# supabase/etl

Measured on AMD Instinct MI355X. Metric: WAL bytes/s decoded, higher is better.
Workload: dtype u8; 1 GPU; cfg2_fixed_5xint4: 64 MiB batches of CopyData-framed pgoutput, device-resident in / device-resident out, offsets sidecar, NO_CONTROL | ASYNC; batch_bytes=67108819, frames_per_batch=594511, pool_batches=6, parallelism=shard1

## Files before the change

### etl_amd/csrc/frames.hip.h

```cpp
#pragma once
#include "values.hip.h"

namespace etlg {

DEV void record_error(const DecParams& p, uint32_t frame, uint32_t rank, uint32_t code) {
  unsigned long long key = ((unsigned long long)frame << 16) | ((unsigned long long)rank << 8) | code;
  atomicMin(&p.res->first_err, key);
}

DEV bool load_carry(DecParams& p) {
  if (!p.carry) return true;
  const bool ok = (p.carry->fused_fail & ~2u) == 0 && p.carry->first_err == kNoErr;
  p.in_txn = p.carry->out_in_txn; p.final_lsn = p.carry->out_final_lsn; p.next_ord = p.carry->out_next_ord;
  if (!ok && blockIdx.x == 0 && threadIdx.x == 0) atomicOr(&p.res->fused_fail, 8u);
  return ok;
}

DEV uint32_t slot_host_id(const DecParams& p, int sl) { return sl >= 0 ? p.slots[sl].host_id : (uint32_t)sl; }

DEV void block_scan3_excl(uint32_t& a, uint32_t& b, uint32_t& c, uint32_t* lds, uint32_t tot[3]) {
  const int lane = threadIdx.x & 63, wave = threadIdx.x >> 6, nw = (int)(blockDim.x >> 6);
  const uint32_t ia = wave_scan_add(a), ib = wave_scan_add(b), ic = wave_scan_add(c);
  if (lane == 63) { lds[3 * wave] = ia; lds[3 * wave + 1] = ib; lds[3 * wave + 2] = ic; }
  __syncthreads();
  uint32_t pa = 0, pb = 0, pc = 0, ta = 0, tb = 0, tc = 0;
  for (int w = 0; w < nw; w++) {
    const uint32_t xa = lds[3 * w], xb = lds[3 * w + 1], xc = lds[3 * w + 2];
    if (w < wave) { pa += xa; pb += xb; pc += xc; }
    ta += xa; tb += xb; tc += xc;
  }
  __syncthreads();
  a = pa + ia - a; b = pb + ib - b; c = pc + ic - c;
  tot[0] = ta; tot[1] = tb; tot[2] = tc;
}

// ... 502 lines not shown
```

### etl_amd/csrc/plan.hip

```cpp
#include "lookback.hip.h"

#ifndef ETLG_PLAN_MINWAVES
#define ETLG_PLAN_MINWAVES 5
#endif

namespace etlg {

struct WinLds {
  const ETLG_LDS_AS u8* base;
  DEV uint32_t w(uint32_t aoff) const { return ETLG_LDS_LD32(base + aoff); }
};
struct WinGlb {
  const u8* base; uint32_t lim;
  DEV uint32_t w(uint32_t aoff) const {
    uint32_t v = 0;
    if (aoff + 4 <= lim) __builtin_memcpy(&v, base + aoff, 4);
    else for (uint32_t k = 0; aoff + k < lim; k++) v |= (uint32_t)base[aoff + k] << (8 * k);
    return v;
  }
};
template <class M> DEV uint32_t rd32(const M& m, uint32_t off) {
  const uint32_t a = off & ~3u, s = off & 3u;
  return __builtin_amdgcn_alignbyte(m.w(a + 4), m.w(a), s);
}
// ... 45 lines not shown
    const uint32_t d2 = dig4(pad_word(__builtin_amdgcn_alignbyte(w3, w2, s), k, 2), bad);
    mag = (uint64_t)d0 * 100000000ull + (d1 * 10000u + d2);
    uint64_t lim;
    if (cls == ETLG_TC_U32) lim = 0xFFFFFFFFull;
    else if (cls == ETLG_TC_I16) lim = neg ? 0x8000ull : 0x7FFFull;
    else lim = neg ? 0x80000000ull : 0x7FFFFFFFull;
    ok = (n != 0u) & (nd != 0u) & (n <= 12u) & (nd <= 11u) & (bad == 0u) & (mag <= lim) & ((cls != ETLG_TC_U32) | (neg ^ 1u));
  }
  return neg ? 0 - mag : mag;
}

DEV int plan_find(const PlanParams& q, uint32_t rel_u) {
  const ETLG_CONST_AS uint32_t* t = (const ETLG_CONST_AS uint32_t*)(uintptr_t)q.tabs;
  int lo = 0, hi = (int)q.n_tabs - 1;
  while (lo <= hi) {
    const int mid = (lo + hi) >> 1;
    const uint32_t v = t[mid * (int)(sizeof(PlanTab) / 4)];
    if (v == rel_u) return mid;
    if (v < rel_u) lo = mid + 1; else hi = mid - 1;
  }
  return -1;
}

#define WSTAMP(k) do { if ((q.dbg & 64u) && threadIdx.x == 0) ((unsigned long long*)p.heap)[(size_t)blockIdx.x * 8 + (k)] = wall_clock64(); } while (0)
#define PSTAMP(k) do { if ((q.dbg & 32u) && threadIdx.x == 0 && (blockIdx.x & 15u) == 3u) { const unsigned long long t_ = clock64(); atomicAdd(&p.res->dbg_t[k], t_ - tprev); tprev = t_; } } while (0)

constexpr uint32_t kPreBeginLen = kBodyOff + 20u, kPreCommitLen = kBodyOff + 25u;
constexpr int kPreTilesPerWave = 8, kPreWaves = 8;
constexpr uint32_t pre_log2(uint32_t v) { return v <= 1u ? 0u : 1u + pre_log2(v >> 1); }
constexpr uint32_t kPreGroupLog = pre_log2(kPreTilesPerWave * kPreWaves);
static_assert((1u << kPreGroupLog) == (uint32_t)(kPreTilesPerWave * kPreWaves), "a group of the pre-pass is a power of two of tiles");
static_assert(kPreTilesPerWave <= 32 && kPreWaves <= 8, "cand_m / short_m are 32-bit masks; at most two waves per SIMD");
constexpr uint32_t kPlanMaxPolls = 1u << 15;

struct PlanPre2 { unsigned long long a0 = 0, l0 = 0, a1 = 0, l1 = 0; bool valid = false; };
struct PlanFold { uint32_t fx, mk, l0, l1; };
DEV PlanFold fold_id() { return PlanFold{0u, 0u, 0u, 0u}; }
DEV PlanFold fold_f(const PlanFold& a, const PlanFold& b) {
  return PlanFold{a.fx + b.fx, a.mk > b.mk ? a.mk : b.mk, b.mk ? b.l0 : a.l0, b.mk ? b.l1 : a.l1};
}
DEV PlanFold fold_of(unsigned long long a, unsigned long long l) {
  return PlanFold{(uint32_t)a, (uint32_t)(a >> 32) & 0x3FFFFFFFu, (uint32_t)l, (uint32_t)(l >> 32) & 0x3FFFFFFFu};
}
DEV unsigned long long fold_agg(const PlanFold& v) { return ((unsigned long long)v.mk << 32) | v.fx; }
DEV unsigned long long fold_lsn(const PlanFold& v) { return ((unsigned long long)v.l1 << 32) | v.l0; }
DEV unsigned long long pair_state(unsigned long long a, unsigned long long l) { const unsigned long long st = a & ST_MASK; return st == (l & ST_MASK) ? st : 0ull; }
DEV PlanFold fold_scan(PlanFold v) {
#define ETLG_P3_DPP(ctrl, rmask) { PlanFold o_; \
// ... 69 lines not shown
    const PlanFold wfold = fold_lane63(fold_scan((int)lane >= (first_incl < 0 ? 0 : first_incl) ? fold_of(wa, wl) : fold_id()));
    acc = fold_f(wfold, acc);
    if (first_incl >= 0) break;
    base -= 64;
  }
  if (j == 63u && lane == 0) { const PlanFold incl = fold_f(acc, group_agg); ETLG_ST_PAIR(g2 + 2 * (size_t)g, ST_INCL | fold_agg(incl), ST_INCL | fold_lsn(incl)); }
  const PlanFold r = fold_f(acc, local);
  ex = fold_agg(r); ex_lsn = fold_lsn(r);
}

template <int RD>
struct PlanLocal {
  uint32_t tbl, slot_id, pm, x_fx, fixed_dw, vbytes, bad;
  uint32_t tagf;
  uint64_t wal_start, b_lsn;
  uint32_t* rimg;
  uint32_t row[RD];
  uint64_t ord;
  uint64_t agg, tile_lsn, ex, ex_lsn, tile_pre_lsn;
  uint32_t tot_mark, tot_fx;
  bool early, done;
};

template <class M, int RD>
DEV void plan_local(const DecParams& p, const PlanParams& q, const M& m, u8* rows, bool stage_own, uint32_t a0, uint32_t tile, uint32_t nt, uint32_t my_o,
                    uint32_t span0, uint32_t span1, unsigned long long& tprev, PlanLocal<RD>& L, bool keep) {
  L.done = true;
  const uint32_t lane = threadIdx.x;
  const bool live = lane < nt;
  const uint32_t f = tile * 64u + lane;
  uint32_t* failp = &p.res->fused_fail;
  uint32_t bad = 0;

  const uint32_t o0 = my_o;
  const uint32_t o1 = (uint32_t)__builtin_amdgcn_update_dpp((int)span1, (int)my_o, 0x130, 0xF, 0xF, false);
  const uint32_t flen = o1 - o0;
  const uint32_t sane = (live ? 1u : 0u) & (o1 > o0) & (o0 >= span0) & (o1 <= span1) & (flen >= 38u);
  bad |= (live ? 1u : 0u) & (sane ^ 1u);
  const uint32_t fr = sane ? o0 - a0 : 0u;
  const uint64_t h30 = rd64(m, fr + 30);
  const uint32_t tag = (uint32_t)(h30 & 0xFF);
  const uint32_t rel = __builtin_bswap32((uint32_t)(h30 >> 8));
  const uint32_t ncols = ((uint32_t)(h30 >> 48) & 0xFFu) << 8 | (uint32_t)(h30 >> 56);
  bad |= sane & (uint32_t)(tag != 'I' && tag != 'U' && tag != 'D' && tag != 'B' && tag != 'C');
  const bool isD = sane && tag == 'D';
  const bool isI = sane && (tag == 'I' || tag == 'U'), isB = sane && tag == 'B', isC = sane && tag == 'C';
  int ti = -1;
  uint32_t row_dw = 0, slot_id = 0, want_cols = 0, key_dw = 0, n_ident = 0;
// ... 13 lines not shown
    }
  }
  bad |= (uint32_t)(isI && (ti < 0 || ncols != want_cols));
  bad |= (uint32_t)(isD && (ti < 0 || key_dw == 0 || (ncols != n_ident && ncols != want_cols)));
  uint64_t b_lsn = 0;
  if (isB) b_lsn = bswap64(rd64(m, fr + 31));
  if (isC) b_lsn = bswap64(rd64(m, fr + 32));
  const uint32_t fixed_dw = isI ? row_dw : isD ? key_dw : isB ? 2u : isC ? 4u : 0u;
  const uint32_t mark = isB ? (((f + 1) << 1) | 1u) : isC ? ((f + 1) << 1) : 0u;
  const uint32_t im = wave_scan_max(mark);
  const uint32_t pm = (uint32_t)__builtin_amdgcn_update_dpp(0, (int)im, 0x138, 0xF, 0xF, false);
  const uint32_t ifx = wave_scan_add(fixed_dw);
  const uint32_t tot_mark = wave_last(im), tot_fx = wave_last(ifx);
  const uint32_t x_fx = ifx - fixed_dw;
  uint64_t tile_lsn = 0;
  if (tot_mark & 1u) {
    const int src = (int)((tot_mark >> 1) - 1u - tile * 64u);
    tile_lsn = ((uint64_t)(uint32_t)__builtin_amdgcn_readlane((int)(uint32_t)(b_lsn >> 32), src) << 32) | (uint32_t)__builtin_amdgcn_readlane((int)(uint32_t)b_lsn, src);
    bad |= (uint32_t)((tile_lsn >> 62) != 0);
    tile_lsn &= ~(3ull << 62);
  }
  PSTAMP(2);
  WSTAMP(2);
  if (q.dbg & 4u) { if (tot_mark + tot_fx == 0xFFFFFFF1u) atomicOr(failp, 2u); return; }

  const uint64_t agg = ((uint64_t)tot_mark << 32) | tot_fx;
  const bool early = (tile & 63u) == 63u;
  uint64_t ex = 0, ex_lsn = 0;
  if (q.pre) bad |= (uint32_t)((isB && flen != kPreBeginLen) || (isC && flen != kPreCommitLen) || (isI && ti >= 0 && (row_dw != q.pre_row_dw || flen < q.pre_key_below)) ||
                               (isD && ti >= 0 && (key_dw != q.pre_key_dw || (flen >= q.pre_key_below && flen > q.pre_key_max))));
  else plan_publish2(q.desc, tile, agg, tile_lsn);
  if (early && !q.pre) plan_resolve2(q.desc, q.desc + 2 * (size_t)q.ntiles, tile, agg, tile_lsn, failp, PlanPre2(), ex, ex_lsn);
  {
    const uint64_t h0 = rd64(m, fr);
    const uint32_t len = __builtin_bswap32((uint32_t)(h0 >> 8));
    const uint32_t env = ((uint32_t)(h0 & 0xFF) == 'd') & (len + 1u == flen) & ((uint32_t)((h0 >> 40) & 0xFF) == 'w');
    const uint32_t shape = (tag == 'I' || tag == 'U') ? (uint32_t)((uint32_t)((h30 >> 40) & 0xFF) == 'N')
                         : tag == 'D' ? (uint32_t)((uint32_t)((h30 >> 40) & 0xFF) == 'K')
                         : tag == 'B' ? (uint32_t)(flen >= kBodyOff + 20) : (uint32_t)(flen >= kBodyOff + 25);
    bad |= sane & ((env & shape) ^ 1u);
  }
  const uint64_t wal_start = bswap64(rd64(m, fr + 6));
  uint64_t b_ts = 0, c_end = 0;
  uint32_t b_xid = 0, c_flags = 0;
  if (isB) { b_ts = bswap64(rd64(m, fr + 39)); b_xid = __builtin_bswap32(rd32(m, fr + 47)); }
  if (isC) { c_flags = (uint32_t)(h30 >> 8) & 0xFFu; c_end = bswap64(rd64(m, fr + 40)); b_ts = bswap64(rd64(m, fr + 48)); }
  uint32_t* rimg = q.lds_bytes > q.rows_off ? (uint32_t*)(rows + q.rows_off) + x_fx : (uint32_t*)(rows + (stage_own ? ((fr + 3u) & ~3u) : lane * 32u));
  if (isB && !bad) { rimg[0] = (uint32_t)b_ts; rimg[1] = (uint32_t)(b_ts >> 32); }
  if (isC && !bad) { rimg[0] = (uint32_t)c_end; rimg[1] = (uint32_t)(c_end >> 32); rimg[2] = (uint32_t)b_ts; rimg[3] = (uint32_t)(b_ts >> 32); }
  uint32_t vbytes = 0;
  if (!(q.dbg & 8u)) {
    unsigned long long todo = __ballot(isI && !bad);
    while (todo) {
      const int leader = __builtin_ctzll(todo);
      const int t_u = __builtin_amdgcn_readlane(ti, leader);
      const bool mine = isI && !bad && ti == t_u;
      const ETLG_CONST_AS uint32_t* tw = (const ETLG_CONST_AS uint32_t*)(uintptr_t)(q.tabs + t_u);
      const uint32_t n_u = tw[2], cb_u = tw[4];
      const ETLG_CONST_AS uint32_t* cw = (const ETLG_CONST_AS uint32_t*)(uintptr_t)(q.cols + cb_u);
      if (mine) {
        uint32_t cur = fr + 38;
        const uint32_t e = fr + flen;
        uint32_t acc = 0, cbad = 0;
        uint32_t cd_next = cw[0];
        for (uint32_t i = 0; i < n_u; i++) {
          const uint32_t cd = cd_next;
          cd_next = cw[i + 1 < n_u ? i + 1 : i];
          const uint32_t cls = cd & 0xFFu;
          uint32_t* slot = rimg + (cd >> 18);
          const uint32_t rc = cur < e ? cur : fr;
          const uint64_t ch = rd64(m, rc);
          const uint32_t kind = (uint32_t)(ch & 0xFF);
          const uint32_t len = __builtin_bswap32((uint32_t)(ch >> 8));
          const uint32_t c0 = (uint32_t)(ch >> 40) & 0xFFu;
// ... 67 lines not shown
            cbad |= fits ^ 1u;
          }
          vbytes += tl;
          cur = rc + (is_t ? 5u + tl : 1u);
        }
        bad |= cbad;
      }
      todo_d &= ~__ballot(mine);
    }
  }
  PSTAMP(3);
  WSTAMP(3);
  L.tbl = isB ? b_xid : (isI || isD) ? rel : 0u; L.slot_id = (isI || isD) ? slot_id : 0u; L.pm = pm; L.x_fx = x_fx; L.fixed_dw = fixed_dw; L.vbytes = vbytes; L.bad = bad;
  if (isD) c_flags = ETLG_OLD_KEY;
  L.tagf = tag | (c_flags << 8) | (((isI || isD) ? 1u : 0u) << 16) | ((isB ? 1u : 0u) << 17) | ((isC ? 1u : 0u) << 18) | ((live ? 1u : 0u) << 19);
  L.wal_start = wal_start; L.b_lsn = b_lsn; L.rimg = rimg;
  if (keep) {
#pragma unroll
    for (int d = 0; d < RD; d++) L.row[d] = rimg[d];
  }
  L.agg = agg; L.tile_lsn = tile_lsn; L.ex = ex; L.ex_lsn = ex_lsn; L.tot_mark = tot_mark; L.tot_fx = tot_fx; L.early = early; L.done = false;
}

DEV void plan_late_carry(DecParams& p, uint32_t* failp) {
  if (!(p.flags & 16u) || !p.carry) return;
  for (uint32_t polls = 0;; polls++) {
    if (__hip_atomic_load(&p.carry->carry_ready, __ATOMIC_ACQUIRE, __HIP_MEMORY_SCOPE_AGENT)) break;
    if (polls > kPlanMaxPolls) { if (threadIdx.x == 0) atomicOr(failp, 1u); break; }
    __builtin_amdgcn_s_sleep(8);
  }
  p.in_txn = __hip_atomic_load(&p.carry->out_in_txn, __ATOMIC_RELAXED, __HIP_MEMORY_SCOPE_AGENT);
  p.final_lsn = __hip_atomic_load(&p.carry->out_final_lsn, __ATOMIC_RELAXED, __HIP_MEMORY_SCOPE_AGENT);
  p.next_ord = __hip_atomic_load(&p.carry->out_next_ord, __ATOMIC_RELAXED, __HIP_MEMORY_SCOPE_AGENT);
  p.flags &= ~16u;
}

struct PlanPreWords { unsigned long long g0 = 0, g1 = 0, t0 = 0, t1 = 0; };
DEV PlanPreWords plan_pre_load(const PlanParams& q, uint32_t tile) {
  PlanPreWords w;
  if (q.pre && tile < q.ntiles) {
    const ETLG_CONST_AS unsigned long long* dt = (const ETLG_CONST_AS unsigned long long*)(uintptr_t)(q.pre + 2 * (size_t)tile);
    const ETLG_CONST_AS unsigned long long* dg = (const ETLG_CONST_AS unsigned long long*)(uintptr_t)(q.pre + 2 * ((size_t)q.ntiles + (tile >> kPreGroupLog)));
    w.t0 = dt[0]; w.t1 = dt[1]; w.g0 = dg[0]; w.g1 = dg[1];
  }
  return w;
}

template <int RD>
DEV void plan_resolve(DecParams& p, const PlanParams& q, uint32_t tile, PlanLocal<RD>& L, unsigned long long& tprev, const PlanPre2& pre = PlanPre2(), const PlanPreWords& pw = PlanPreWords()) {
  if (L.done) return;
  const uint32_t lane = threadIdx.x;
  const uint32_t f = tile * 64u + lane;
  uint32_t* failp = &p.res->fused_fail;
  uint32_t bad = L.bad;
  const bool isI = (L.tagf >> 16) & 1u, isB = (L.tagf >> 17) & 1u, isC = (L.tagf >> 18) & 1u;
  const uint32_t pm = L.pm;
  const uint64_t b_lsn = L.b_lsn;
  uint64_t ex = L.ex, ex_lsn = L.ex_lsn;

  if (q.pre) {
    const PlanFold r = fold_f(fold_of(pw.g0, pw.g1), fold_of(pw.t0, pw.t1));
    ex = fold_agg(r); ex_lsn = fold_lsn(r);
  }
  else if (!L.early) plan_resolve2(q.desc, q.desc + 2 * (size_t)q.ntiles, tile, L.agg, L.tile_lsn, failp, pre, ex, ex_lsn);
  PSTAMP(7);
  uint32_t pre_mark = (uint32_t)(ex >> 32);
  if (pre_mark == 0) {
    plan_late_carry(p, failp);
    if (p.in_txn) { pre_mark = 1u; ex |= 1ull << 32; }
  }
  const uint64_t pre_lsn = (pre_mark & 1u) && (pre_mark >> 1) != 0 ? ex_lsn : p.final_lsn;
  PSTAMP(4);
  WSTAMP(4);

  const uint32_t last = pre_mark > pm ? pre_mark : pm;
  const bool in_txn = (last & 1u) != 0;
  const uint32_t fb1 = last >> 1;
  uint64_t final_lsn = 0;
  {
    const bool here = in_txn && fb1 != 0 && fb1 - 1 >= tile * 64u;
    const uint32_t src = here ? fb1 - 1 - tile * 64u : 0u;
    const uint32_t lo = (uint32_t)__shfl((int)(uint32_t)b_lsn, (int)src, 64), hi = (uint32_t)__shfl((int)(uint32_t)(b_lsn >> 32), (int)src, 64);
    if (in_txn) final_lsn = here ? (((uint64_t)hi << 32) | lo) : pre_lsn;
  }
  uint64_t ord = 0;
  if (!isB && in_txn) ord = fb1 == 0 ? p.next_ord + f : (uint64_t)(f - (fb1 - 1));
  bad |= (uint32_t)((isI || isC) && !in_txn);
  bad |= (uint32_t)(isC && in_txn && b_lsn != final_lsn);
  L.bad = bad; L.ex = ex; L.tile_pre_lsn = pre_lsn;
  L.b_lsn = isI ? final_lsn : b_lsn;
  L.ord = ord;
}

template <bool REGS, int RD>
DEV void plan_store(DecParams& p, const PlanParams& q, uint32_t tile, const PlanLocal<RD>& L, unsigned long long& tprev) {
  if (L.done) return;
  const uint32_t lane = threadIdx.x;
  const uint32_t f = tile * 64u + lane;
  uint32_t* failp = &p.res->fused_fail;
  const uint32_t bad = L.bad;
  const uint32_t tag = L.tagf & 0xFFu, c_flags = (L.tagf >> 8) & 0xFFu;
  const bool live = (L.tagf >> 19) & 1u;
  const uint32_t x_fx = L.x_fx, fixed_dw = L.fixed_dw, vbytes = L.vbytes, tot_mark = L.tot_mark, tot_fx = L.tot_fx;
  const uint64_t tile_lsn = L.tile_lsn, pre_lsn = L.tile_pre_lsn;
  const uint32_t pre_mark = (uint32_t)(L.ex >> 32);
  const uint64_t pre_fx = (uint64_t)(uint32_t)L.ex << 2;

  if (tile == q.ntiles - 1 && lane == 0) {
    DevResult* r = p.res;
    r->n_events = p.nframes; r->fixed_bytes = pre_fx + ((uint64_t)tot_fx << 2); r->heap_bytes = 0; r->n_frames = p.nframes;
    const uint32_t lm = pre_mark > tot_mark ? pre_mark : tot_mark;
    const bool it = (lm & 1u) != 0;
    r->out_in_txn = it;
    uint64_t fl = 0, no = 0;
    if (it) {
      const uint32_t lb1 = lm >> 1;
      fl = tot_mark ? tile_lsn : pre_lsn;
      no = lb1 == 0 ? p.next_ord + p.nframes : (uint64_t)(p.nframes - (lb1 - 1));
    }
    r->out_final_lsn = fl; r->out_next_ord = no;
    __hip_atomic_store(&r->carry_ready, 1u, __ATOMIC_RELEASE, __HIP_MEMORY_SCOPE_AGENT);
  }

  const uint64_t fx_off = pre_fx + ((uint64_t)x_fx << 2);
  const uint32_t any_bad = __any(bad != 0u) ? 1u : 0u;
  const bool cap_ok = pre_fx + ((uint64_t)tot_fx << 2) <= p.fixed_cap;
  if (!any_bad && cap_ok && !(q.dbg & 8u)) {
    uint32_t* dst = (uint32_t*)(p.fixed + fx_off);
    if (REGS) {
#pragma unroll
      for (uint32_t d = 0; d < (uint32_t)RD; d++) if (d < fixed_dw) dst[d] = L.row[d];
    } else {
      const uint32_t* rimg = L.rimg;
      for (uint32_t d = 0; d < fixed_dw; d++) dst[d] = rimg[d];
    }
  }
  PSTAMP(5);
  if (live && !any_bad && cap_ok && !(q.dbg & 16u)) {
    p.ev_kind[f] = (u8)tag;
    p.ev_flags[f] = (u8)c_flags;
    p.ev_table[f] = L.tbl;
    p.ev_slot[f] = L.slot_id;
    p.ev_start[f] = L.wal_start;
    p.ev_commit[f] = L.b_lsn;
    p.ev_ord[f] = L.ord;
    p.ev_body[f] = fx_off;
  }
  PSTAMP(6);
  WSTAMP(5);
  const bool is_upd = (L.tagf & 0xFFu) == 'U', is_del = (L.tagf & 0xFFu) == 'D';
  const uint32_t pay = wave_last(wave_scan_add((is_upd || is_del) ? 0u : vbytes));
  if (lane == 0 && pay) atomicAdd(&p.res->pay_shard[tile & 31][0], (unsigned long long)pay);
  if (__ballot(is_upd && vbytes != 0)) {
    const uint32_t payu = wave_last(wave_scan_add(is_upd ? vbytes : 0u));
    if (lane == 0 && payu) atomicAdd(&p.res->pay_shard[tile & 31][1], (unsigned long long)payu);
  }
  if (__ballot(is_del && vbytes != 0)) {
    const uint32_t payd = wave_last(wave_scan_add(is_del ? vbytes : 0u));
    if (lane == 0 && payd) atomicAdd(&p.res->pay_shard[tile & 31][2], (unsigned long long)payd);
  }
  if ((any_bad || !cap_ok) && lane == 0) atomicOr(failp, 2u);
}

struct TileSpan { uint32_t nt, span0, span1, my_o; };
DEV TileSpan plan_span(const DecParams& p, uint32_t tile) {
  const uint32_t lane = threadIdx.x;
  TileSpan t;
  const uint32_t f0 = tile * 64u;
  t.nt = p.nframes - f0 < 64u ? p.nframes - f0 : 64u;
  const ETLG_CONST_AS uint32_t* offs_c = (const ETLG_CONST_AS uint32_t*)(uintptr_t)p.offs;
  t.span0 = offs_c[f0]; t.span1 = offs_c[f0 + t.nt];
  t.my_o = lane < t.nt ? p.offs[f0 + lane] : t.span1;
  return t;
}

template <int RD>
DEV void plan_stage_local(DecParams& p, const PlanParams& q, u8* smem, uint32_t tile, const TileSpan& ts, unsigned long long& tprev, PlanLocal<RD>& L, bool keep) {
  const uint32_t lane = threadIdx.x;
  L.done = true;
  const uint32_t nt = ts.nt, span0 = ts.span0, span1 = ts.span1, my_o = ts.my_o;
  PSTAMP(0);
  const uint32_t a0 = span0 & ~15u;
  const bool staged = span1 > span0 && span1 <= p.in_len && (uint64_t)(span1 - a0) + 64 <= q.rows_off && !(q.dbg & 1u);
  if (staged) {
    const uint32_t npieces = (span1 - a0 + 1023u) >> 10;
    for (uint32_t k = 0; k < npieces; k++) {
      const uint32_t c = a0 + (k << 10) + (lane << 4);
      if (c < span1 && (uint64_t)c + 16 <= p.in_len) ETLG_GLDS16(p.in + c, smem + (k << 10));
    }
    const uint32_t tail = a0 + (((uint32_t)p.in_len - a0) & ~15u);
    if (tail < span1 && (uint64_t)tail + 16 > p.in_len && tail + lane < p.in_len && lane < 16) smem[tail - a0 + lane] = p.in[tail + lane];
    ETLG_VMEM_WAIT();
    PSTAMP(1);
    WSTAMP(1);
    if (q.dbg & 2u) { if (smem[lane * 97u] == 0xEE && smem[lane * 13u + 5u] == 0xEF && my_o == 0xFFFFFFF1u) atomicOr(&p.res->fused_fail, 2u); return; }
    const WinLds m{(const ETLG_LDS_AS u8*)smem};
    plan_local(p, q, m, smem, true, a0, tile, nt, my_o, span0, span1, tprev, L, keep);
  } else {
    const WinGlb m{p.in, (uint32_t)p.in_len};
    plan_local(p, q, m, smem, false, 0u, tile, nt, my_o, span0, span1, tprev, L, keep);
  }
}

DEV bool plan_frames_from_device(DecParams& p, PlanParams& q) {
  if (!p.nframes_dev) return true;
  const ETLG_CONST_AS uint32_t* r = (const ETLG_CONST_AS uint32_t*)(uintptr_t)p.nframes_dev;
  const uint32_t nf = r[0], flags = r[1] | r[2];
  if (flags != 0 || nf == 0 || nf > p.nframes) {
    if (blockIdx.x == 0 && threadIdx.x == 0) {
      atomicOr(&p.res->fused_fail, 32u);
      __hip_atomic_store(&p.res->carry_ready, 1u, __ATOMIC_RELEASE, __HIP_MEMORY_SCOPE_AGENT);
    }
    return false;
  }
  p.nframes = nf;
  q.ntiles = (nf + 63u) >> 6;
  return true;
}

template <bool TWO, int RD>
DEV void plan_kernel(DecParams& p, const PlanParams& q_in, u8* smem) {
  PlanParams q = q_in;
  const uint32_t lane = threadIdx.x;
  unsigned long long tprev = (q.dbg & 32u) ? clock64() : 0ull;
  const uint32_t tile = blockIdx.x;
  WSTAMP(0);
  clear_next_descriptors<64>(q.d_clear, q.clear_words, lane);
  if (!(p.flags & 16u) && !load_carry(p)) return;
  if (!plan_frames_from_device(p, q)) return;
  const uint32_t t0 = TWO ? 2u * blockIdx.x : blockIdx.x;
  if (t0 >= q.ntiles) return;
  const TileSpan sa = plan_span(p, t0);
  const PlanPreWords pwa = plan_pre_load(q, t0), pwb = TWO ? plan_pre_load(q, t0 + 1u) : PlanPreWords();
  TileSpan sb = sa;
  if (TWO && t0 + 1u < q.ntiles) sb = plan_span(p, t0 + 1u);
  PlanLocal<RD> A;
  plan_stage_local(p, q, smem, t0, sa, tprev, A, TWO);
  if (TWO) {
    const uint32_t t1 = t0 + 1u;
    PlanLocal<RD> B;
    B.done = true;
    if (t1 < q.ntiles) {
      __threadfence_block();
      __syncthreads();
      plan_stage_local(p, q, smem, t1, sb, tprev, B, false);
    }
    PlanPre2 preA, preB;
    if (!A.done && !A.early && !q.pre) preA = plan_prefetch2(q.desc, q.desc + 2 * (size_t)q.ntiles, t0);
    if (!B.done && !B.early && !q.pre) preB = plan_prefetch2(q.desc, q.desc + 2 * (size_t)q.ntiles, t1);
    plan_resolve(p, q, t0, A, tprev, preA, pwa);
    plan_resolve(p, q, t1, B, tprev, preB, pwb);
    plan_store<true>(p, q, t0, A, tprev);
    plan_store<false>(p, q, t1, B, tprev);
  } else {
    plan_resolve(p, q, t0, A, tprev, PlanPre2(), pwa);
    plan_store<false>(p, q, t0, A, tprev);
  }
}

__global__ __launch_bounds__(kPreWaves * 64) void k_plan_pre(DecParams p, PlanParams q) {
  __shared__ unsigned long long s_wagg[kPreWaves][2];
  if (!plan_frames_from_device(p, q)) return;
  if (blockIdx.x >= ((q.ntiles + (1u << kPreGroupLog) - 1u) >> kPreGroupLog)) return;
  const uint32_t lane = threadIdx.x & 63u, wave = (uint32_t)__builtin_amdgcn_readfirstlane((int)(threadIdx.x >> 6)), g = blockIdx.x;
  const uint32_t t0 = (g << kPreGroupLog) + wave * (uint32_t)kPreTilesPerWave;
  uint32_t o[kPreTilesPerWave + 1];
#pragma unroll
  for (int i = 0; i <= kPreTilesPerWave; i++) {
    const uint64_t f = (uint64_t)(t0 + (uint32_t)i) * 64u + lane;
    o[i] = p.offs[f < p.nframes ? f : p.nframes];
  }
  uint32_t cand_m = 0;
  uint32_t short_m = 0;
  uint32_t tagv[kPreTilesPerWave];
  uint64_t lsnv[kPreTilesPerWave];
#pragma unroll
  for (int i = 0; i < kPreTilesPerWave; i++) {
    const uint64_t f = (uint64_t)(t0 + (uint32_t)i) * 64u + lane;
    const uint32_t o0 = o[i];
// ... 66 lines not shown
    unsigned long long a = gi < ng ? na : tagbits, l = gi < ng ? nl : tagbits;
    if (gi + 64u < ng) ETLG_LD_PAIR(gd + 2 * (size_t)(gi + 64u), na, nl);
    bool have = pair_state(a, l) == tagbits;
    bool gave_up = false;
    for (uint32_t polls = 0;; polls++) {
      if (!have) { ETLG_LD_PAIR(gd + 2 * (size_t)gi, a, l); have = pair_state(a, l) == tagbits; }
      if (!__ballot(!have)) break;
      if (polls > kPlanMaxPolls) { if (lane == 0) atomicOr(&p.res->fused_fail, 1u); gave_up = true; break; }
      __builtin_amdgcn_s_sleep(2);
    }
    const PlanFold inc = fold_scan(gi < ng ? fold_of(a, l) : fold_id());
    PlanFold exc;
    exc.fx = (uint32_t)__builtin_amdgcn_update_dpp(0, (int)inc.fx, 0x138, 0xF, 0xF, false); exc.mk = (uint32_t)__builtin_amdgcn_update_dpp(0, (int)inc.mk, 0x138, 0xF, 0xF, false);
    exc.l0 = (uint32_t)__builtin_amdgcn_update_dpp(0, (int)inc.l0, 0x138, 0xF, 0xF, false); exc.l1 = (uint32_t)__builtin_amdgcn_update_dpp(0, (int)inc.l1, 0x138, 0xF, 0xF, false);
    const PlanFold r = fold_f(carry, exc);
    if (gi < ng && !gave_up) { gd[2 * (size_t)gi] = fold_agg(r); gd[2 * (size_t)gi + 1] = fold_lsn(r); }
    carry = fold_f(carry, fold_lane63(inc));
  }
  if (lane == 0) __hip_atomic_store(q.pre_ticket, 0u, __ATOMIC_RELAXED, __HIP_MEMORY_SCOPE_AGENT);
}

__global__ __launch_bounds__(64, ETLG_PLAN_MINWAVES) void k_plan(DecParams p, PlanParams q) {
  ETLG_DYNAMIC_LDS(smem);
  plan_kernel<false, 1>(p, q, smem);
}

template <int RD>
__global__ __launch_bounds__(64, ETLG_PLAN_MINWAVES) void k_plan2(DecParams p, PlanParams q) {
  ETLG_DYNAMIC_LDS(smem);
  plan_kernel<true, RD>(p, q, smem);
}

}

extern "C" {

using namespace etlg;

void etlg_k_launch_plan_pre(const DecParams* p, const PlanParams* q, hipStream_t s) {
  hipLaunchKernelGGL(k_plan_pre, dim3((q->ntiles + (1u << kPreGroupLog) - 1u) >> kPreGroupLog), dim3(kPreWaves * 64), 0, s, *p, *q);
}

void etlg_k_launch_plan(const DecParams* p, const PlanParams* q, hipStream_t s) {
  if (q->lds_bytes == q->rows_off && q->max_row_dw <= 8u && !(q->dbg & 512u)) {
    if (q->max_row_dw <= 6u) hipLaunchKernelGGL(k_plan2<6>, dim3((q->ntiles + 1) / 2), dim3(64), q->lds_bytes, s, *p, *q);
    else hipLaunchKernelGGL(k_plan2<8>, dim3((q->ntiles + 1) / 2), dim3(64), q->lds_bytes, s, *p, *q);
  } else hipLaunchKernelGGL(k_plan, dim3(q->ntiles), dim3(64), q->lds_bytes, s, *p, *q);
}

uint32_t etlg_k_plan_pre_group_log(void) { return kPreGroupLog; }

int etlg_k_plan_set_lds(void) {
  const int a = hipFuncSetAttribute((const void*)k_plan, hipFuncAttributeMaxDynamicSharedMemorySize, 64 * 1024) == hipSuccess ? 0 : 1;
  const int b = hipFuncSetAttribute((const void*)k_plan2<6>, hipFuncAttributeMaxDynamicSharedMemorySize, 64 * 1024) == hipSuccess ? 0 : 1;
  const int c = hipFuncSetAttribute((const void*)k_plan2<8>, hipFuncAttributeMaxDynamicSharedMemorySize, 64 * 1024) == hipSuccess ? 0 : 1;
  return a | b | c;
}

}
```

Before: 1861 GB/s.

## Split plan kernel into debug and non-debug variants and hoist prologue loads

```diff
diff --git a/etl_amd/csrc/frames.hip.h b/etl_amd/csrc/frames.hip.h
--- a/etl_amd/csrc/frames.hip.h
+++ b/etl_amd/csrc/frames.hip.h
@@ -8,9 +8,10 @@
   atomicMin(&p.res->first_err, key);
 }
 
+DEV bool carry_usable(uint32_t fused_fail, unsigned long long first_err) { return (fused_fail & ~2u) == 0 && first_err == kNoErr; }
 DEV bool load_carry(DecParams& p) {
   if (!p.carry) return true;
-  const bool ok = (p.carry->fused_fail & ~2u) == 0 && p.carry->first_err == kNoErr;
+  const bool ok = carry_usable(p.carry->fused_fail, p.carry->first_err);
   p.in_txn = p.carry->out_in_txn; p.final_lsn = p.carry->out_final_lsn; p.next_ord = p.carry->out_next_ord;
   if (!ok && blockIdx.x == 0 && threadIdx.x == 0) atomicOr(&p.res->fused_fail, 8u);
   return ok;
diff --git a/etl_amd/csrc/plan.hip b/etl_amd/csrc/plan.hip
--- a/etl_amd/csrc/plan.hip
+++ b/etl_amd/csrc/plan.hip
@@ -91,8 +91,11 @@
   return -1;
 }
 
-#define WSTAMP(k) do { if ((q.dbg & 64u) && threadIdx.x == 0) ((unsigned long long*)p.heap)[(size_t)blockIdx.x * 8 + (k)] = wall_clock64(); } while (0)
-#define PSTAMP(k) do { if ((q.dbg & 32u) && threadIdx.x == 0 && (blockIdx.x & 15u) == 3u) { const unsigned long long t_ = clock64(); atomicAdd(&p.res->dbg_t[k], t_ - tprev); tprev = t_; } } while (0)
+template <bool DBG> DEV bool plan_dbg(const PlanParams& q, uint32_t bits) {
+  if constexpr (DBG) return (q.dbg & bits) != 0u; else return false;
+}
+#define WSTAMP(k) do { if constexpr (DBG) { if ((q.dbg & 64u) && threadIdx.x == 0) ((unsigned long long*)p.heap)[(size_t)blockIdx.x * 8 + (k)] = wall_clock64(); } } while (0)
+#define PSTAMP(k) do { if constexpr (DBG) { if ((q.dbg & 32u) && threadIdx.x == 0 && (blockIdx.x & 15u) == 3u) { const unsigned long long t_ = clock64(); atomicAdd(&p.res->dbg_t[k], t_ - tprev); tprev = t_; } } } while (0)
 
 constexpr uint32_t kPreBeginLen = kBodyOff + 20u, kPreCommitLen = kBodyOff + 25u;
 constexpr int kPreTilesPerWave = 8, kPreWaves = 8;
@@ -208,8 +211,8 @@
   bool early, done;
 };
 
-template <class M, int RD>
-DEV void plan_local(const DecParams& p, const PlanParams& q, const M& m, u8* rows, bool stage_own, uint32_t a0, uint32_t tile, uint32_t nt, uint32_t my_o,
+template <bool DBG, class M, int RD>
+DEV void plan_local(const DecParams& p, const PlanParams& q, uint32_t ntiles, const M& m, u8* rows, bool stage_own, uint32_t a0, uint32_t tile, uint32_t nt, uint32_t my_o,
                     uint32_t span0, uint32_t span1, unsigned long long& tprev, PlanLocal<RD>& L, bool keep) {
   L.done = true;
   const uint32_t lane = threadIdx.x;
@@ -269,7 +272,7 @@
   }
   PSTAMP(2);
   WSTAMP(2);
-  if (q.dbg & 4u) { if (tot_mark + tot_fx == 0xFFFFFFF1u) atomicOr(failp, 2u); return; }
+  if (plan_dbg<DBG>(q, 4u)) { if (lane == 0) atomicOr(failp, tot_mark + tot_fx == 0xFFFFFFF1u ? 3u : 2u); return; }
 
   const uint64_t agg = ((uint64_t)tot_mark << 32) | tot_fx;
   const bool early = (tile & 63u) == 63u;
@@ -277,7 +280,7 @@
   if (q.pre) bad |= (uint32_t)((isB && flen != kPreBeginLen) || (isC && flen != kPreCommitLen) || (isI && ti >= 0 && (row_dw != q.pre_row_dw || flen < q.pre_key_below)) ||
                                (isD && ti >= 0 && (key_dw != q.pre_key_dw || (flen >= q.pre_key_below && flen > q.pre_key_max))));
   else plan_publish2(q.desc, tile, agg, tile_lsn);
-  if (early && !q.pre) plan_resolve2(q.desc, q.desc + 2 * (size_t)q.ntiles, tile, agg, tile_lsn, failp, PlanPre2(), ex, ex_lsn);
+  if (early && !q.pre) plan_resolve2(q.desc, q.desc + 2 * (size_t)ntiles, tile, agg, tile_lsn, failp, PlanPre2(), ex, ex_lsn);
   {
     const uint64_t h0 = rd64(m, fr);
     const uint32_t len = __builtin_bswap32((uint32_t)(h0 >> 8));
@@ -296,7 +299,7 @@
   if (isB && !bad) { rimg[0] = (uint32_t)b_ts; rimg[1] = (uint32_t)(b_ts >> 32); }
   if (isC && !bad) { rimg[0] = (uint32_t)c_end; rimg[1] = (uint32_t)(c_end >> 32); rimg[2] = (uint32_t)b_ts; rimg[3] = (uint32_t)(b_ts >> 32); }
   uint32_t vbytes = 0;
-  if (!(q.dbg & 8u)) {
+  if (!plan_dbg<DBG>(q, 8u)) {
     unsigned long long todo = __ballot(isI && !bad);
     while (todo) {
       const int leader = __builtin_ctzll(todo);
@@ -410,32 +413,47 @@
   L.agg = agg; L.tile_lsn = tile_lsn; L.ex = ex; L.ex_lsn = ex_lsn; L.tot_mark = tot_mark; L.tot_fx = tot_fx; L.early = early; L.done = false;
 }
 
-DEV void plan_late_carry(DecParams& p, uint32_t* failp) {
-  if (!(p.flags & 16u) || !p.carry) return;
+struct PlanBatch {
+  uint32_t nframes, ntiles, in_txn;
+  uint64_t final_lsn, next_ord;
+  const DevResult* carry;
+  bool late;
+};
+DEV void plan_late_carry(PlanBatch& b, uint32_t* failp) {
+  if (!b.late) return;
   for (uint32_t polls = 0;; polls++) {
-    if (__hip_atomic_load(&p.carry->carry_ready, __ATOMIC_ACQUIRE, __HIP_MEMORY_SCOPE_AGENT)) break;
+    if (__hip_atomic_load(&b.carry->carry_ready, __ATOMIC_ACQUIRE, __HIP_MEMORY_SCOPE_AGENT)) break;
     if (polls > kPlanMaxPolls) { if (threadIdx.x == 0) atomicOr(failp, 1u); break; }
     __builtin_amdgcn_s_sleep(8);
   }
-  p.in_txn = __hip_atomic_load(&p.carry->out_in_txn, __ATOMIC_RELAXED, __HIP_MEMORY_SCOPE_AGENT);
-  p.final_lsn = __hip_atomic_load(&p.carry->out_final_lsn, __ATOMIC_RELAXED, __HIP_MEMORY_SCOPE_AGENT);
-  p.next_ord = __hip_atomic_load(&p.carry->out_next_ord, __ATOMIC_RELAXED, __HIP_MEMORY_SCOPE_AGENT);
-  p.flags &= ~16u;
+  b.in_txn = __hip_atomic_load(&b.carry->out_in_txn, __ATOMIC_RELAXED, __HIP_MEMORY_SCOPE_AGENT);
+  b.final_lsn = __hip_atomic_load(&b.carry->out_final_lsn, __ATOMIC_RELAXED, __HIP_MEMORY_SCOPE_AGENT);
+  b.next_ord = __hip_atomic_load(&b.carry->out_next_ord, __ATOMIC_RELAXED, __HIP_MEMORY_SCOPE_AGENT);
+  b.late = false;
 }
 
 struct PlanPreWords { unsigned long long g0 = 0, g1 = 0, t0 = 0, t1 = 0; };
-DEV PlanPreWords plan_pre_load(const PlanParams& q, uint32_t tile) {
+DEV uint32_t plan_pre_load(const unsigned long long* pre, uint32_t ntiles, uint32_t tile0) {
+  const uint32_t lane = threadIdx.x, tile = tile0 + (lane >> 3);
+  uint32_t v = 0;
+  if (pre && lane < 16u && tile < ntiles) {
+    const unsigned long long* w = pre + 2 * ((lane & 4u) ? (size_t)ntiles + (tile >> kPreGroupLog) : (size_t)tile);
+    v = ((const uint32_t*)w)[lane & 3u];
+  }
+  return v;
+}
+DEV PlanPreWords plan_pre_words(uint32_t v, int which) {
+  uint32_t d[8];
+#pragma unroll
+  for (int i = 0; i < 8; i++) d[i] = (uint32_t)__builtin_amdgcn_readlane((int)v, 8 * which + i);
   PlanPreWords w;
-  if (q.pre && tile < q.ntiles) {
-    const ETLG_CONST_AS unsigned long long* dt = (const ETLG_CONST_AS unsigned long long*)(uintptr_t)(q.pre + 2 * (size_t)tile);
-    const ETLG_CONST_AS unsigned long long* dg = (const ETLG_CONST_AS unsigned long long*)(uintptr_t)(q.pre + 2 * ((size_t)q.ntiles + (tile >> kPreGroupLog)));
-    w.t0 = dt[0]; w.t1 = dt[1]; w.g0 = dg[0]; w.g1 = dg[1];
-  }
+  w.t0 = ((unsigned long long)d[1] << 32) | d[0]; w.t1 = ((unsigned long long)d[3] << 32) | d[2];
+  w.g0 = ((unsigned long long)d[5] << 32) | d[4]; w.g1 = ((unsigned long long)d[7] << 32) | d[6];
   return w;
 }
 
-template <int RD>
-DEV void plan_resolve(DecParams& p, const PlanParams& q, uint32_t tile, PlanLocal<RD>& L, unsigned long long& tprev, const PlanPre2& pre = PlanPre2(), const PlanPreWords& pw = PlanPreWords()) {
+template <bool DBG, int RD>
+DEV void plan_resolve(const DecParams& p, const PlanParams& q, PlanBatch& b, uint32_t tile, PlanLocal<RD>& L, unsigned long long& tprev, const PlanPre2& pre, uint32_t pre_v, int which) {
   if (L.done) return;
   const uint32_t lane = threadIdx.x;
   const uint32_t f = tile * 64u + lane;
@@ -447,17 +465,18 @@
   uint64_t ex = L.ex, ex_lsn = L.ex_lsn;
 
   if (q.pre) {
+    const PlanPreWords pw = plan_pre_words(pre_v, which);
     const PlanFold r = fold_f(fold_of(pw.g0, pw.g1), fold_of(pw.t0, pw.t1));
     ex = fold_agg(r); ex_lsn = fold_lsn(r);
   }
-  else if (!L.early) plan_resolve2(q.desc, q.desc + 2 * (size_t)q.ntiles, tile, L.agg, L.tile_lsn, failp, pre, ex, ex_lsn);
+  else if (!L.early) plan_resolve2(q.desc, q.desc + 2 * (size_t)b.ntiles, tile, L.agg, L.tile_lsn, failp, pre, ex, ex_lsn);
   PSTAMP(7);
   uint32_t pre_mark = (uint32_t)(ex >> 32);
   if (pre_mark == 0) {
-    plan_late_carry(p, failp);
-    if (p.in_txn) { pre_mark = 1u; ex |= 1ull << 32; }
-  }
-  const uint64_t pre_lsn = (pre_mark & 1u) && (pre_mark >> 1) != 0 ? ex_lsn : p.final_lsn;
+    plan_late_carry(b, failp);
+    if (b.in_txn) { pre_mark = 1u; ex |= 1ull << 32; }
+  }
+  const uint64_t pre_lsn = (pre_mark & 1u) && (pre_mark >> 1) != 0 ? ex_lsn : b.final_lsn;
   PSTAMP(4);
   WSTAMP(4);
 
@@ -472,7 +491,7 @@
     if (in_txn) final_lsn = here ? (((uint64_t)hi << 32) | lo) : pre_lsn;
   }
   uint64_t ord = 0;
-  if (!isB && in_txn) ord = fb1 == 0 ? p.next_ord + f : (uint64_t)(f - (fb1 - 1));
+  if (!isB && in_txn) ord = fb1 == 0 ? b.next_ord + f : (uint64_t)(f - (fb1 - 1));
   bad |= (uint32_t)((isI || isC) && !in_txn);
   bad |= (uint32_t)(isC && in_txn && b_lsn != final_lsn);
   L.bad = bad; L.ex = ex; L.tile_pre_lsn = pre_lsn;
@@ -480,8 +499,8 @@
   L.ord = ord;
 }
 
-template <bool REGS, int RD>
-DEV void plan_store(DecParams& p, const PlanParams& q, uint32_t tile, const PlanLocal<RD>& L, unsigned long long& tprev) {
+template <bool DBG, bool REGS, int RD>
+DEV void plan_store(const DecParams& p, const PlanParams& q, const PlanBatch& b, uint32_t tile, const PlanLocal<RD>& L, unsigned long long& tprev) {
   if (L.done) return;
   const uint32_t lane = threadIdx.x;
   const uint32_t f = tile * 64u + lane;
@@ -494,9 +513,9 @@
   const uint32_t pre_mark = (uint32_t)(L.ex >> 32);
   const uint64_t pre_fx = (uint64_t)(uint32_t)L.ex << 2;
 
-  if (tile == q.ntiles - 1 && lane == 0) {
+  if (tile == b.ntiles - 1 && lane == 0) {
     DevResult* r = p.res;
-    r->n_events = p.nframes; r->fixed_bytes = pre_fx + ((uint64_t)tot_fx << 2); r->heap_bytes = 0; r->n_frames = p.nframes;
+    r->n_events = b.nframes; r->fixed_bytes = pre_fx + ((uint64_t)tot_fx << 2); r->heap_bytes = 0; r->n_frames = b.nframes;
     const uint32_t lm = pre_mark > tot_mark ? pre_mark : tot_mark;
     const bool it = (lm & 1u) != 0;
     r->out_in_txn = it;
@@ -504,7 +523,7 @@
     if (it) {
       const uint32_t lb1 = lm >> 1;
       fl = tot_mark ? tile_lsn : pre_lsn;
-      no = lb1 == 0 ? p.next_ord + p.nframes : (uint64_t)(p.nframes - (lb1 - 1));
+      no = lb1 == 0 ? b.next_ord + b.nframes : (uint64_t)(b.nframes - (lb1 - 1));
     }
     r->out_final_lsn = fl; r->out_next_ord = no;
     __hip_atomic_store(&r->carry_ready, 1u, __ATOMIC_RELEASE, __HIP_MEMORY_SCOPE_AGENT);
@@ -513,7 +532,7 @@
   const uint64_t fx_off = pre_fx + ((uint64_t)x_fx << 2);
   const uint32_t any_bad = __any(bad != 0u) ? 1u : 0u;
   const bool cap_ok = pre_fx + ((uint64_t)tot_fx << 2) <= p.fixed_cap;
-  if (!any_bad && cap_ok && !(q.dbg & 8u)) {
+  if (!any_bad && cap_ok && !plan_dbg<DBG>(q, 8u)) {
     uint32_t* dst = (uint32_t*)(p.fixed + fx_off);
     if (REGS) {
 #pragma unroll
@@ -524,7 +543,7 @@
     }
   }
   PSTAMP(5);
-  if (live && !any_bad && cap_ok && !(q.dbg & 16u)) {
+  if (live && !any_bad && cap_ok && !plan_dbg<DBG>(q, 16u)) {
     p.ev_kind[f] = (u8)tag;
     p.ev_flags[f] = (u8)c_flags;
     p.ev_table[f] = L.tbl;
@@ -550,99 +569,190 @@
   if ((any_bad || !cap_ok) && lane == 0) atomicOr(failp, 2u);
 }
 
+
 struct TileSpan { uint32_t nt, span0, span1, my_o; };
-DEV TileSpan plan_span(const DecParams& p, uint32_t tile) {
+DEV TileSpan plan_span(const uint32_t* offs, uint32_t nframes, uint32_t tile) {
   const uint32_t lane = threadIdx.x;
   TileSpan t;
   const uint32_t f0 = tile * 64u;
-  t.nt = p.nframes - f0 < 64u ? p.nframes - f0 : 64u;
-  const ETLG_CONST_AS uint32_t* offs_c = (const ETLG_CONST_AS uint32_t*)(uintptr_t)p.offs;
+  t.nt = nframes - f0 < 64u ? nframes - f0 : 64u;
+  const ETLG_CONST_AS uint32_t* offs_c = (const ETLG_CONST_AS uint32_t*)(uintptr_t)offs;
   t.span0 = offs_c[f0]; t.span1 = offs_c[f0 + t.nt];
-  t.my_o = lane < t.nt ? p.offs[f0 + lane] : t.span1;
+  t.my_o = offs[f0 + (lane < t.nt ? lane : t.nt)];
   return t;
 }
-
-template <int RD>
-DEV void plan_stage_local(DecParams& p, const PlanParams& q, u8* smem, uint32_t tile, const TileSpan& ts, unsigned long long& tprev, PlanLocal<RD>& L, bool keep) {
+struct TileSpanB { uint32_t nt, ends, my_o; };
+DEV TileSpanB plan_span_b(const uint32_t* offs, uint32_t nframes, uint32_t tile) {
+  const uint32_t lane = threadIdx.x;
+  TileSpanB t;
+  const uint32_t f0 = tile * 64u;
+  t.nt = nframes - f0 < 64u ? nframes - f0 : 64u;
+  t.ends = offs[f0 + (lane ? t.nt : 0u)];
+  t.my_o = offs[f0 + (lane < t.nt ? lane : t.nt)];
+  return t;
+}
+DEV TileSpan plan_span_of(const TileSpanB& s) {
+  return TileSpan{s.nt, (uint32_t)__builtin_amdgcn_readlane((int)s.ends, 0), (uint32_t)__builtin_amdgcn_readlane((int)s.ends, 1), s.my_o};
+}
+
+struct PlanCarry { unsigned long long first_err = kNoErr; uint32_t fused_fail = 0, in_txn = 0; uint64_t final_lsn = 0, next_ord = 0; };
+DEV PlanCarry plan_carry_load(const DevResult* carry) {
+  const ETLG_CONST_AS DevResult* c = (const ETLG_CONST_AS DevResult*)(uintptr_t)carry;
+  PlanCarry w;
+  w.first_err = c->first_err; w.fused_fail = c->fused_fail; w.in_txn = c->out_in_txn; w.final_lsn = c->out_final_lsn; w.next_ord = c->out_next_ord;
+  return w;
+}
+DEV void plan_carry_failed(DevResult* res) { if (blockIdx.x == 0 && threadIdx.x == 0) atomicOr(&res->fused_fail, 8u); }
+
+struct PlanDevCount { uint32_t nf = 0, flags = 0; };
+DEV PlanDevCount plan_count_load(const uint32_t* nframes_dev) {
+  const ETLG_CONST_AS uint32_t* r = (const ETLG_CONST_AS uint32_t*)(uintptr_t)nframes_dev;
+  PlanDevCount c;
+  c.nf = r[0]; c.flags = r[1] | r[2];
+  return c;
+}
+DEV bool plan_count_ok(const PlanDevCount& c, uint32_t bound) { return c.flags == 0 && c.nf != 0 && c.nf <= bound; }
+DEV void plan_count_failed(DevResult* res) {
+  if (blockIdx.x == 0 && threadIdx.x == 0) {
+    atomicOr(&res->fused_fail, 32u);
+    __hip_atomic_store(&res->carry_ready, 1u, __ATOMIC_RELEASE, __HIP_MEMORY_SCOPE_AGENT);
+  }
+}
+DEV bool plan_frames_from_device(DecParams& p, PlanParams& q) {
+  if (!p.nframes_dev) return true;
+  const PlanDevCount c = plan_count_load(p.nframes_dev);
+  if (!plan_count_ok(c, p.nframes)) { plan_count_failed(p.res); return false; }
+  p.nframes = c.nf;
+  q.ntiles = (c.nf + 63u) >> 6;
+  return true;
+}
+
+struct PlanStage { uint32_t a0; bool staged; };
+template <bool DBG>
+DEV PlanStage plan_stage_issue(const DecParams& p, const PlanParams& q, const u8* in, uint64_t in_len, u8* smem, const TileSpan& ts, unsigned long long& tprev) {
+  const uint32_t lane = threadIdx.x;
+  const uint32_t span0 = ts.span0, span1 = ts.span1;
+  PSTAMP(0);
+  PlanStage g;
+  g.a0 = span0 & ~15u;
+  g.staged = span1 > span0 && span1 <= in_len && (uint64_t)(span1 - g.a0) + 64 <= q.rows_off && !plan_dbg<DBG>(q, 1u);
+  if (g.staged) {
+    const uint32_t a0 = g.a0, npieces = (span1 - a0 + 1023u) >> 10;
+    for (uint32_t k = 0; k < npieces; k++) {
+      const uint32_t c = a0 + (k << 10) + (lane << 4);
+      if (c < span1 && (uint64_t)c + 16 <= in_len) ETLG_GLDS16(in + c, smem + (k << 10));
+    }
+    const uint32_t tail = a0 + (((uint32_t)in_len - a0) & ~15u);
+    if (tail < span1 && (uint64_t)tail + 16 > in_len && tail + lane < in_len && lane < 16) smem[tail - a0 + lane] = in[tail + lane];
+  }
+  return g;
+}
+
+template <bool DBG, int RD>
+DEV void plan_stage_local(const DecParams& p, const PlanParams& q, uint32_t ntiles, const u8* in, uint64_t in_len, u8* smem, uint32_t tile, const TileSpan& ts,
+                          const PlanStage& g, unsigned long long& tprev, PlanLocal<RD>& L, bool keep) {
   const uint32_t lane = threadIdx.x;
   L.done = true;
   const uint32_t nt = ts.nt, span0 = ts.span0, span1 = ts.span1, my_o = ts.my_o;
-  PSTAMP(0);
-  const uint32_t a0 = span0 & ~15u;
-  const bool staged = span1 > span0 && span1 <= p.in_len && (uint64_t)(span1 - a0) + 64 <= q.rows_off && !(q.dbg & 1u);
-  if (staged) {
-    const uint32_t npieces = (span1 - a0 + 1023u) >> 10;
-    for (uint32_t k = 0; k < npieces; k++) {
-      const uint32_t c = a0 + (k << 10) + (lane << 4);
-      if (c < span1 && (uint64_t)c + 16 <= p.in_len) ETLG_GLDS16(p.in + c, smem + (k << 10));
-    }
-    const uint32_t tail = a0 + (((uint32_t)p.in_len - a0) & ~15u);
-    if (tail < span1 && (uint64_t)tail + 16 > p.in_len && tail + lane < p.in_len && lane < 16) smem[tail - a0 + lane] = p.in[tail + lane];
+  if (g.staged) {
     ETLG_VMEM_WAIT();
     PSTAMP(1);
     WSTAMP(1);
-    if (q.dbg & 2u) { if (smem[lane * 97u] == 0xEE && smem[lane * 13u + 5u] == 0xEF && my_o == 0xFFFFFFF1u) atomicOr(&p.res->fused_fail, 2u); return; }
+    if (plan_dbg<DBG>(q, 2u)) {
+      const bool odd = smem[lane * 97u] == 0xEE && smem[lane * 13u + 5u] == 0xEF && my_o == 0xFFFFFFF1u;
+      if (__any(odd) || lane == 0) atomicOr(&p.res->fused_fail, 2u);
+      return;
+    }
     const WinLds m{(const ETLG_LDS_AS u8*)smem};
-    plan_local(p, q, m, smem, true, a0, tile, nt, my_o, span0, span1, tprev, L, keep);
+    plan_local<DBG>(p, q, ntiles, m, smem, true, g.a0, tile, nt, my_o, span0, span1, tprev, L, keep);
   } else {
-    const WinGlb m{p.in, (uint32_t)p.in_len};
-    plan_local(p, q, m, smem, false, 0u, tile, nt, my_o, span0, span1, tprev, L, keep);
-  }
-}
-
-DEV bool plan_frames_from_device(DecParams& p, PlanParams& q) {
-  if (!p.nframes_dev) return true;
-  const ETLG_CONST_AS uint32_t* r = (const ETLG_CONST_AS uint32_t*)(uintptr_t)p.nframes_dev;
-  const uint32_t nf = r[0], flags = r[1] | r[2];
-  if (flags != 0 || nf == 0 || nf > p.nframes) {
-    if (blockIdx.x == 0 && threadIdx.x == 0) {
-      atomicOr(&p.res->fused_fail, 32u);
-      __hip_atomic_store(&p.res->carry_ready, 1u, __ATOMIC_RELEASE, __HIP_MEMORY_SCOPE_AGENT);
-    }
-    return false;
-  }
-  p.nframes = nf;
-  q.ntiles = (nf + 63u) >> 6;
-  return true;
-}
-
-template <bool TWO, int RD>
-DEV void plan_kernel(DecParams& p, const PlanParams& q_in, u8* smem) {
-  PlanParams q = q_in;
+    const WinGlb m{in, (uint32_t)in_len};
+    plan_local<DBG>(p, q, ntiles, m, smem, false, 0u, tile, nt, my_o, span0, span1, tprev, L, keep);
+  }
+}
+
+#ifdef ETLG_SIMT
+#define PLAN_HOLD_ARGS(...) ((void)0)
+#define PLAN_HOLD_DATA(a0, a1, cw) ((void)0)
+#define PLAN_HOLD_COUNT(dc) ((void)0)
+#else
+#define PLAN_HOLD_ARGS(in, offs, in_len, nf_dev, pre, carry, res, flags, nframes, ntiles, rows_off, n_tabs, in_txn, final_lsn, next_ord, tabs, cols, pre_row_dw, \
+                       pre_key_dw, pre_key_below, pre_key_max, fixed, fixed_cap) \
+  asm volatile("" :: "s"(in), "s"(offs), "s"(in_len), "s"(nf_dev), "s"(pre), "s"(carry), "s"(res), "s"(flags), "s"(nframes), "s"(ntiles), "s"(rows_off), "s"(n_tabs), \
+               "s"(in_txn), "s"(final_lsn), "s"(next_ord), "s"(tabs), "s"(cols), "s"(pre_row_dw), "s"(pre_key_dw), "s"(pre_key_below), "s"(pre_key_max), "s"(fixed), "s"(fixed_cap))
+#define PLAN_HOLD_DATA(a0, a1, cw) \
+  asm volatile("" :: "s"(a0), "s"(a1), "s"(cw.first_err), "s"(cw.fused_fail), "s"(cw.in_txn), "s"(cw.final_lsn), "s"(cw.next_ord))
+#define PLAN_HOLD_COUNT(dc) asm volatile("" :: "s"(dc.nf), "s"(dc.flags))
+#endif
+
+template <bool TWO, int RD, bool DBG>
+DEV void plan_kernel(const DecParams& p, const PlanParams& q, u8* smem) {
   const uint32_t lane = threadIdx.x;
-  unsigned long long tprev = (q.dbg & 32u) ? clock64() : 0ull;
-  const uint32_t tile = blockIdx.x;
+  const u8* const in = p.in;
+  const uint32_t* const offs = p.offs;
+  const uint64_t in_len = p.in_len;
+  const uint32_t* const nf_dev = p.nframes_dev;
+  const unsigned long long* const pre = q.pre;
+  const DevResult* const carry = p.carry;
+  DevResult* const res = p.res;
+  const uint32_t flags = p.flags, nframes = p.nframes, ntiles = q.ntiles, rows_off = q.rows_off, n_tabs = q.n_tabs, in_txn = p.in_txn;
+  const uint64_t final_lsn = p.final_lsn, next_ord = p.next_ord;
+  PLAN_HOLD_ARGS(in, offs, in_len, nf_dev, pre, carry, res, flags, nframes, ntiles, rows_off, n_tabs, in_txn, final_lsn, next_ord, q.tabs, q.cols, q.pre_row_dw,
+                 q.pre_key_dw, q.pre_key_below, q.pre_key_max, p.fixed, p.fixed_cap);
+  const bool carry_now = !(flags & 16u) && carry != nullptr;
+  PlanBatch b{nframes, ntiles, in_txn, final_lsn, next_ord, carry, (flags & 16u) != 0u && carry != nullptr};
+  unsigned long long tprev = 0ull;
+  if constexpr (DBG) tprev = (q.dbg & 32u) ? clock64() : 0ull;
   WSTAMP(0);
+  const uint32_t t0 = TWO ? 2u * blockIdx.x : blockIdx.x;
+  if (nf_dev) {
+    const PlanDevCount dc = plan_count_load(nf_dev);
+    PlanCarry cw;
+    if (carry_now) cw = plan_carry_load(carry);
+    PLAN_HOLD_COUNT(dc);
+    if (carry_now && !carry_usable(cw.fused_fail, cw.first_err)) { plan_carry_failed(res); clear_next_descriptors<64>(q.d_clear, q.clear_words, lane); return; }
+    if (!plan_count_ok(dc, b.nframes)) { plan_count_failed(res); clear_next_descriptors<64>(q.d_clear, q.clear_words, lane); return; }
+    b.nframes = dc.nf;
+    b.ntiles = (dc.nf + 63u) >> 6;
+  }
+  if (t0 >= b.ntiles) { clear_next_descriptors<64>(q.d_clear, q.clear_words, lane); return; }
+  const bool two = TWO && t0 + 1u < b.ntiles;
+  const TileSpan sa = plan_span(offs, b.nframes, t0);
+  TileSpanB sbv{};
+  if constexpr (TWO) sbv = plan_span_b(offs, b.nframes, two ? t0 + 1u : t0);
+  const uint32_t pre_v = plan_pre_load(pre, b.ntiles, t0);
+  PlanCarry cw;
+  if (carry_now) cw = plan_carry_load(carry);
+  PLAN_HOLD_DATA(sa.span0, sa.span1, cw);
+  if (carry_now) {
+    if (!carry_usable(cw.fused_fail, cw.first_err)) { plan_carry_failed(res); clear_next_descriptors<64>(q.d_clear, q.clear_words, lane); return; }
+    b.in_txn = cw.in_txn; b.final_lsn = cw.final_lsn; b.next_ord = cw.next_ord;
+  }
+  PlanLocal<RD> A;
+  const PlanStage ga = plan_stage_issue<DBG>(p, q, in, in_len, smem, sa, tprev);
   clear_next_descriptors<64>(q.d_clear, q.clear_words, lane);
-  if (!(p.flags & 16u) && !load_carry(p)) return;
-  if (!plan_frames_from_device(p, q)) return;
-  const uint32_t t0 = TWO ? 2u * blockIdx.x : blockIdx.x;
-  if (t0 >= q.ntiles) return;
-  const TileSpan sa = plan_span(p, t0);
-  const PlanPreWords pwa = plan_pre_load(q, t0), pwb = TWO ? plan_pre_load(q, t0 + 1u) : PlanPreWords();
-  TileSpan sb = sa;
-  if (TWO && t0 + 1u < q.ntiles) sb = plan_span(p, t0 + 1u);
-  PlanLocal<RD> A;
-  plan_stage_local(p, q, smem, t0, sa, tprev, A, TWO);
+  plan_stage_local<DBG>(p, q, b.ntiles, in, in_len, smem, t0, sa, ga, tprev, A, TWO);
   if (TWO) {
     const uint32_t t1 = t0 + 1u;
     PlanLocal<RD> B;
     B.done = true;
-    if (t1 < q.ntiles) {
+    if (two) {
       __threadfence_block();
       __syncthreads();
-      plan_stage_local(p, q, smem, t1, sb, tprev, B, false);
+      const TileSpan sb = plan_span_of(sbv);
+      const PlanStage gb = plan_stage_issue<DBG>(p, q, in, in_len, smem, sb, tprev);
+      plan_stage_local<DBG>(p, q, b.ntiles, in, in_len, smem, t1, sb, gb, tprev, B, false);
     }
     PlanPre2 preA, preB;
-    if (!A.done && !A.early && !q.pre) preA = plan_prefetch2(q.desc, q.desc + 2 * (size_t)q.ntiles, t0);
-    if (!B.done && !B.early && !q.pre) preB = plan_prefetch2(q.desc, q.desc + 2 * (size_t)q.ntiles, t1);
-    plan_resolve(p, q, t0, A, tprev, preA, pwa);
-    plan_resolve(p, q, t1, B, tprev, preB, pwb);
-    plan_store<true>(p, q, t0, A, tprev);
-    plan_store<false>(p, q, t1, B, tprev);
+    if (!A.done && !A.early && !pre) preA = plan_prefetch2(q.desc, q.desc + 2 * (size_t)b.ntiles, t0);
+    if (!B.done && !B.early && !pre) preB = plan_prefetch2(q.desc, q.desc + 2 * (size_t)b.ntiles, t1);
+    plan_resolve<DBG>(p, q, b, t0, A, tprev, preA, pre_v, 0);
+    plan_resolve<DBG>(p, q, b, t1, B, tprev, preB, pre_v, 1);
+    plan_store<DBG, true>(p, q, b, t0, A, tprev);
+    plan_store<DBG, false>(p, q, b, t1, B, tprev);
   } else {
-    plan_resolve(p, q, t0, A, tprev, PlanPre2(), pwa);
-    plan_store<false>(p, q, t0, A, tprev);
+    plan_resolve<DBG>(p, q, b, t0, A, tprev, PlanPre2(), pre_v, 0);
+    plan_store<DBG, false>(p, q, b, t0, A, tprev);
   }
 }
 
@@ -755,13 +865,24 @@
 
 __global__ __launch_bounds__(64, ETLG_PLAN_MINWAVES) void k_plan(DecParams p, PlanParams q) {
   ETLG_DYNAMIC_LDS(smem);
-  plan_kernel<false, 1>(p, q, smem);
+  plan_kernel<false, 1, false>(p, q, smem);
 }
 
 template <int RD>
 __global__ __launch_bounds__(64, ETLG_PLAN_MINWAVES) void k_plan2(DecParams p, PlanParams q) {
   ETLG_DYNAMIC_LDS(smem);
-  plan_kernel<true, RD>(p, q, smem);
+  plan_kernel<true, RD, false>(p, q, smem);
+}
+
+__global__ __launch_bounds__(64, ETLG_PLAN_MINWAVES) void k_plan_dbg(DecParams p, PlanParams q) {
+  ETLG_DYNAMIC_LDS(smem);
+  plan_kernel<false, 1, true>(p, q, smem);
+}
+
+template <int RD>
+__global__ __launch_bounds__(64, ETLG_PLAN_MINWAVES) void k_plan2_dbg(DecParams p, PlanParams q) {
+  ETLG_DYNAMIC_LDS(smem);
+  plan_kernel<true, RD, true>(p, q, smem);
 }
 
 }
@@ -775,19 +896,27 @@
 }
 
 void etlg_k_launch_plan(const DecParams* p, const PlanParams* q, hipStream_t s) {
-  if (q->lds_bytes == q->rows_off && q->max_row_dw <= 8u && !(q->dbg & 512u)) {
-    if (q->max_row_dw <= 6u) hipLaunchKernelGGL(k_plan2<6>, dim3((q->ntiles + 1) / 2), dim3(64), q->lds_bytes, s, *p, *q);
-    else hipLaunchKernelGGL(k_plan2<8>, dim3((q->ntiles + 1) / 2), dim3(64), q->lds_bytes, s, *p, *q);
-  } else hipLaunchKernelGGL(k_plan, dim3(q->ntiles), dim3(64), q->lds_bytes, s, *p, *q);
+  const bool two = q->lds_bytes == q->rows_off && q->max_row_dw <= 8u && !(q->dbg & 512u), dbg = (q->dbg & ~512u) != 0u;
+  const dim3 grid(two ? (q->ntiles + 1) / 2 : q->ntiles);
+  if (!dbg) {
+    if (!two) hipLaunchKernelGGL(k_plan, grid, dim3(64), q->lds_bytes, s, *p, *q);
+    else if (q->max_row_dw <= 6u) hipLaunchKernelGGL(k_plan2<6>, grid, dim3(64), q->lds_bytes, s, *p, *q);
+    else hipLaunchKernelGGL(k_plan2<8>, grid, dim3(64), q->lds_bytes, s, *p, *q);
+  } else {
+    if (!two) hipLaunchKernelGGL(k_plan_dbg, grid, dim3(64), q->lds_bytes, s, *p, *q);
+    else if (q->max_row_dw <= 6u) hipLaunchKernelGGL(k_plan2_dbg<6>, grid, dim3(64), q->lds_bytes, s, *p, *q);
+    else hipLaunchKernelGGL(k_plan2_dbg<8>, grid, dim3(64), q->lds_bytes, s, *p, *q);
+  }
 }
 
 uint32_t etlg_k_plan_pre_group_log(void) { return kPreGroupLog; }
 
 int etlg_k_plan_set_lds(void) {
-  const int a = hipFuncSetAttribute((const void*)k_plan, hipFuncAttributeMaxDynamicSharedMemorySize, 64 * 1024) == hipSuccess ? 0 : 1;
-  const int b = hipFuncSetAttribute((const void*)k_plan2<6>, hipFuncAttributeMaxDynamicSharedMemorySize, 64 * 1024) == hipSuccess ? 0 : 1;
-  const int c = hipFuncSetAttribute((const void*)k_plan2<8>, hipFuncAttributeMaxDynamicSharedMemorySize, 64 * 1024) == hipSuccess ? 0 : 1;
-  return a | b | c;
-}
-
-}
+  const void* const kernels[] = {(const void*)k_plan, (const void*)k_plan2<6>, (const void*)k_plan2<8>,
+                                 (const void*)k_plan_dbg, (const void*)k_plan2_dbg<6>, (const void*)k_plan2_dbg<8>};
+  int bad = 0;
+  for (const void* k : kernels) bad |= hipFuncSetAttribute(k, hipFuncAttributeMaxDynamicSharedMemorySize, 64 * 1024) == hipSuccess ? 0 : 1;
+  return bad;
+}
+
+}
```

Measured after the change: 1922 GB/s, median of 6. 3.3% higher.
